# mitake/k8s

Hardware: AMD Instinct MI355X
Metric: images/sec ResNet-50 TfJob (train, synthetic ImageNet) (higher is better)
Workload: dtype bf16; 1 GPU; model=resnet50-v1.5, global_batch=3072, per_gpu_batch=3072, image_size=224, parallelism=dp1, optimizer=fused SGD momentum 0.9 (HIP)

## Files before the change

### k8s_amd/csrc/kernels/conv3x3.hip

```cpp
#include <stdexcept>

#include "common.h"
#include "launchers.h"
#include "mfma.h"

namespace k8s_amd {

namespace c3 {
constexpr int THREADS = 256;
constexpr int STAT_REPL = 32;
__device__ __attribute__((aligned(64))) uint16_t g_c3_zero[64];

__device__ __forceinline__ int swz(int p) { return p & 6; }

__device__ __forceinline__ void raw_barrier() {
  asm volatile("" ::: "memory");
  __builtin_amdgcn_s_barrier();
  asm volatile("" ::: "memory");
}

template <int W, int RT, int KT, bool XF>
struct Geo {
  static constexpr int WP = (W + 7) / 8 * 8 + (W % 8 == 0 ? 8 : 0), P = RT * W;
  static constexpr int NPOS = (RT + 2) * WP + 8;
  static constexpr int MF = (P + 31) / 32, NF = KT / 32;
  static constexpr int WIN_B = NPOS * 128, WT_B = KT * 128;
  static constexpr int NS = WIN_B + 3 * WT_B <= 80 * 1024 ? 3 : 2;
  static constexpr int STAGE_B = 32 * MF * KT * 2;
  static constexpr int LDS = (WIN_B + NS * WT_B) > STAGE_B ? (WIN_B + NS * WT_B) : STAGE_B;
  static_assert(WIN_B + NS * WT_B <= 80 * 1024, "two blocks per CU");
  static_assert(LDS >= THREADS * 16 * 4, "room for the statistics partials");
  static_assert(WP % 8 == 0 && WP > W, "pitch");
};

template <int W, int RT, int KT, bool XF>
__global__ void __launch_bounds__(THREADS, 2) conv3x3_kernel(const uint16_t* __restrict__ x,
                                                            const uint16_t* __restrict__ wt, uint16_t* __restrict__ y,
                                                            float* __restrict__ stats, const float* __restrict__ xf,
                                                            int H, int C, int K, int tiles_per_img, BnBwdSums bb) {
  using G = Geo<W, RT, KT, XF>;
  constexpr int WP = G::WP, NPOS = G::NPOS, P = G::P, MF = G::MF, NF = G::NF, NS = G::NS;
  constexpr int WOPS = KT * 8 / THREADS;
  __shared__ __attribute__((aligned(1024))) char smem[G::LDS];
  char* const win = smem;
  const int tid = threadIdx.x, lane = tid & 63;
  const int wid = __builtin_amdgcn_readfirstlane(tid >> 6);
  const int wm = wid >> 1, wn = wid & 1;
  const int tile = blockIdx.x;
  const int n = tile / tiles_per_img, h0 = (tile - n * tiles_per_img) * RT;
  const int k0 = blockIdx.y * KT;

  int pw[MF];
#pragma unroll
  for (int f = 0; f < MF; ++f) {
    const int m = (wm * MF + f) * 16 + (lane & 15), r = m / W;
    pw[f] = r * WP + 7 + (m - r * W);
  }
  int boff[2][NF];
#pragma unroll
  for (int kk = 0; kk < 2; ++kk)
#pragma unroll
    for (int j = 0; j < NF; ++j) {
      const int r = wn * (KT / 2) + j * 16 + (lane & 15), ch = kk * 4 + (lane >> 4);
      boff[kk][j] = r * 128 + ((ch ^ swz(r)) << 4);
    }
  f32x4_t acc[MF][NF];
#pragma unroll
  for (int f = 0; f < MF; ++f)
#pragma unroll
    for (int j = 0; j < NF; ++j) acc[f][j] = f32x4_t{0.f, 0.f, 0.f, 0.f};

  constexpr int PADR = WP - W, NPAD = 8 + (RT + 2) * PADR;
#pragma unroll
  for (int t0 = 0; t0 < NPAD * 8; t0 += THREADS) {
    const int t = t0 + tid, pi = t >> 3;
    if (t < NPAD * 8) {
      const int r = (pi - 8) / PADR;
      const int pos = pi < 8 ? pi : 8 + r * WP + W + (pi - 8 - r * PADR);
      *reinterpret_cast<bf16x8_t*>(win + (pos * 8 + (t & 7)) * 16) = bf16x8_t{0, 0, 0, 0, 0, 0, 0, 0};
    }
  }
  constexpr int IPR = (W * 8 + 63) / 64, NWI = (RT + 2) * IPR;
  const int lch = (lane & 7) ^ ((lane >> 3) & 6);
  const uint16_t* const xlane = x + ((long)n * H * W + (lane >> 3)) * C + lch * 8;
  auto load_window = [&](int c0) {
#pragma unroll 1
    for (int wi = wid; wi < NWI; wi += THREADS / 64) {
      const int wr = wi / IPR, i = wi - wr * IPR, h = h0 - 1 + wr;
      if (i * 8 + (lane >> 3) < W) {
        const void* src = (unsigned)h < (unsigned)H ? (const void*)(xlane + (h * W + i * 8) * C + c0)
                                                    : (const void*)g_c3_zero;
        glds16(src, win + (wr * WP + 8 + i * 8) * 128);
      }
    }
  };
  auto transform_window = [&](int c0) {
    const int lc = (tid & 7) ^ ((tid >> 3) & 6);
    float sc[8], sh[8];
#pragma unroll
    for (int j = 0; j < 8; ++j) {
      sc[j] = xf[c0 + lc * 8 + j];
      sh[j] = xf[C + c0 + lc * 8 + j];
    }
#pragma unroll 1
    for (int c = tid; c < NPOS * 8; c += THREADS) {
      const int q = (c >> 3) - 8, wr = q / WP, h = h0 - 1 + wr;
      if (q >= 0 && q - wr * WP < W && wr < RT + 2 && (unsigned)h < (unsigned)H) {
        bf16x8_t* qp = reinterpret_cast<bf16x8_t*>(win + c * 16);
        const bf16x8_t v = *qp;
        float o[8];
#pragma unroll
        for (int j = 0; j < 8; ++j) o[j] = fmaxf(__builtin_fmaf(bf2f((uint16_t)v[j]), sc[j], sh[j]), 0.f);
        *qp = pack_bf16x8(o);
      }
    }
    __syncthreads();
  };
  uint32_t wlane[WOPS];
#pragma unroll
  for (int i = 0; i < WOPS; ++i) {
    const int c = i * THREADS + tid, row = c >> 3, lc = (c & 7) ^ swz(row);
    wlane[i] = (uint32_t)(((k0 + row) * 9 * C + lc * 8) * 2);
  }
  auto stage_w = [&](int tap, int c0, int slot) {
    char* d = smem + G::WIN_B + slot * G::WT_B;
#pragma unroll
    for (int i = 0; i < WOPS; ++i) {
      glds16(reinterpret_cast<const char*>(wt + tap * C + c0) + wlane[i], d + (i * THREADS + wid * 64) * 16);
    }
  };
  auto tap_of = [](int k) { return (k % 3) * 3 + k / 3; };

  constexpr int CPR = KT / 8;
  constexpr int RSTEP = THREADS / CPR, NR = (P + RSTEP - 1) / RSTEP;
  constexpr bool XEARLY = KT == 64;
  const int c = tid % CPR, row0 = tid / CPR;
  const bool bst = bb.sums != nullptr;
  bf16x8_t xr[NR];
  auto load_xr = [&]() {
#pragma unroll
    for (int i = 0; i < NR; ++i) {
      const int m = row0 + i * RSTEP, hr = m / W, h = h0 + hr;
      xr[i] = bf16x8_t{0, 0, 0, 0, 0, 0, 0, 0};
      if (m < P && h < H)
        xr[i] = *reinterpret_cast<const bf16x8_t*>(bb.x + (((long)n * H + h) * W + (m - hr * W)) * K + k0 + c * 8);
    }
  };
  const int nsteps = (C >> 6) * 9;
  load_window(0);
  if (XEARLY && bst) load_xr();
#pragma unroll
  for (int g = 0; g < NS - 1; ++g)
    if (g < nsteps) stage_w(tap_of(g), 0, g);
  asm volatile("s_waitcnt vmcnt(0)" ::: "memory");
  __syncthreads();
  if constexpr (XF) transform_window(0);
#pragma unroll 1
  for (int cs = 0; cs < (C >> 6); ++cs) {
    if (cs) {
      load_window(cs * 64);
      asm volatile("s_waitcnt vmcnt(0)" ::: "memory");
      __syncthreads();
      if constexpr (XF) transform_window(cs * 64);
    }
#pragma unroll 1
    for (int ds = 0; ds < 3; ++ds) {
      int aoff[2][MF];
#pragma unroll
      for (int f = 0; f < MF; ++f) {
        const int p = pw[f] + ds;
#pragma unroll
        for (int kk = 0; kk < 2; ++kk) aoff[kk][f] = p * 128 + (((kk * 4 + (lane >> 4)) ^ swz(p)) << 4);
      }
#pragma unroll
      for (int dr = 0; dr < 3; ++dr) {
        const int g = cs * 9 + ds * 3 + dr, gp = g + NS - 1;
        if (gp < nsteps) stage_w(tap_of(gp % 9), gp / 9 * 64, gp % NS);
        const char* ws = smem + G::WIN_B + (NS == 3 ? dr : g & 1) * G::WT_B;
        const char* wa = win + dr * WP * 128;
        if constexpr (NF == 2) {
          mfma_bf16x8 af[2][MF], bfr[2][NF];
#pragma unroll
          for (int kk = 0; kk < 2; ++kk) {
#pragma unroll
            for (int f = 0; f < MF; ++f)
              af[kk][f] = __builtin_bit_cast(mfma_bf16x8, *reinterpret_cast<const bf16x8_t*>(wa + aoff[kk][f]));
#pragma unroll
            for (int j = 0; j < NF; ++j)
              bfr[kk][j] = __builtin_bit_cast(mfma_bf16x8, *reinterpret_cast<const bf16x8_t*>(ws + boff[kk][j]));
          }
          __builtin_amdgcn_sched_barrier(0);
#pragma unroll
          for (int kk = 0; kk < 2; ++kk) {
            if (kk == 0) asm volatile("s_waitcnt lgkmcnt(%0)" ::"n"(MF + NF) : "memory");
            else asm volatile("s_waitcnt lgkmcnt(0)" ::: "memory");
            __builtin_amdgcn_sched_barrier(0);
#pragma unroll
            for (int f = 0; f < MF; ++f)
#pragma unroll
              for (int j = 0; j < NF; ++j)
                acc[f][j] = __builtin_amdgcn_mfma_f32_16x16x32_bf16(bfr[kk][j], af[kk][f], acc[f][j], 0, 0, 0);
            __builtin_amdgcn_sched_barrier(0);
          }
        } else {
#pragma unroll
          for (int kk = 0; kk < 2; ++kk) {
            mfma_bf16x8 af[MF], bfr[NF];
#pragma unroll
            for (int f = 0; f < MF; ++f)
              af[f] = __builtin_bit_cast(mfma_bf16x8, *reinterpret_cast<const bf16x8_t*>(wa + aoff[kk][f]));
#pragma unroll
            for (int j = 0; j < NF; ++j)
              bfr[j] = __builtin_bit_cast(mfma_bf16x8, *reinterpret_cast<const bf16x8_t*>(ws + boff[kk][j]));
#pragma unroll
            for (int f = 0; f < MF; ++f)
#pragma unroll
              for (int j = 0; j < NF; ++j)
                acc[f][j] = __builtin_amdgcn_mfma_f32_16x16x32_bf16(bfr[j], af[f], acc[f][j], 0, 0, 0);
          }
        }
        if (NS > 2 && gp < nsteps) asm volatile("s_waitcnt vmcnt(%0)" ::"n"(WOPS * (NS - 2)) : "memory");
        else asm volatile("s_waitcnt vmcnt(0)" ::: "memory");
        asm volatile("s_waitcnt lgkmcnt(0)" ::: "memory");
        raw_barrier();
      }
    }
  }

  float bsc[8], bsh[8], bmu[8];
  if (bst) {
#pragma unroll
    for (int j = 0; j < 8; ++j) {
      const int col = k0 + c * 8 + j;
      bmu[j] = bb.mean[col];
      bn_affine_regs(bb.gamma[col], bb.beta[col], bmu[j], bb.invstd[col], bsc[j], bsh[j]);
    }
    if (!XEARLY) load_xr();
  }
  uint16_t* const ctile = reinterpret_cast<uint16_t*>(smem);
#pragma unroll
  for (int f = 0; f < MF; ++f) {
    const int row = (wm * MF + f) * 16 + (lane & 15);
#pragma unroll
    for (int j = 0; j < NF; ++j) {
      const int col = wn * (KT / 2) + j * 16 + (lane >> 4) * 4;
      const bf16x4_t o = __builtin_bit_cast(bf16x4_t, __builtin_convertvector(acc[f][j], bf16v4_t));
      *reinterpret_cast<bf16x4_t*>(ctile + row * KT + (((col >> 3) ^ (row % CPR)) << 3) + (col & 4)) = o;
    }
  }
  __syncthreads();
  f32x2_t s2[4], q2[4];
#pragma unroll
  for (int r = 0; r < 4; ++r) s2[r] = q2[r] = f32x2_t{0.f, 0.f};
  if (bst) {
#pragma unroll
    for (int i = 0; i < NR; ++i) {
      const int m = row0 + i * RSTEP, hr = m / W, h = h0 + hr;
      if (m < P && h < H) {
        const bf16x8_t o = *reinterpret_cast<const bf16x8_t*>(ctile + m * KT + ((c ^ (m % CPR)) << 3));
        *reinterpret_cast<bf16x8_t*>(y + (((long)n * H + h) * W + (m - hr * W)) * K + k0 + c * 8) = o;
#pragma unroll
        for (int r = 0; r < 4; ++r) {
          f32x2_t g, d;
#pragma unroll
          for (int e = 0; e < 2; ++e) {
            const float xv = bf2f((uint16_t)xr[i][2 * r + e]);
            g[e] = relu_on(xv, bsc[2 * r + e], bsh[2 * r + e]) ? bf2f((uint16_t)o[2 * r + e]) : 0.f;
            d[e] = xv - bmu[2 * r + e];
          }
          s2[r] += g;
          q2[r] = __builtin_elementwise_fma(g, d, q2[r]);
        }
      }
    }
  } else {
#pragma unroll 2
  for (int m = row0; m < P; m += RSTEP) {
    const int hr = m / W, h = h0 + hr;
    if (h < H) {
      const bf16x8_t o = *reinterpret_cast<const bf16x8_t*>(ctile + m * KT + ((c ^ (m % CPR)) << 3));
      *reinterpret_cast<bf16x8_t*>(y + (((long)n * H + h) * W + (m - hr * W)) * K + k0 + c * 8) = o;
      if (stats) {
        const uint32_t* w = reinterpret_cast<const uint32_t*>(&o);
#pragma unroll
        for (int r = 0; r < 4; ++r) {
          const f32x2_t v = {__uint_as_float(w[r] << 16), __uint_as_float(w[r] & 0xFFFF0000u)};
          s2[r] += v;
          q2[r] = __builtin_elementwise_fma(v, v, q2[r]);
        }
      }
    }
  }
  }
  if (stats || bst) {
    __syncthreads();
    float* part = reinterpret_cast<float*>(smem);
#pragma unroll
    for (int r = 0; r < 4; ++r) {
      part[tid * 16 + 2 * r] = s2[r][0];
      part[tid * 16 + 2 * r + 1] = s2[r][1];
      part[tid * 16 + 8 + 2 * r] = q2[r][0];
      part[tid * 16 + 8 + 2 * r + 1] = q2[r][1];
    }
    __syncthreads();
    if (tid < 2 * KT) {
      const int col = tid % KT, which = tid / KT, cc = col >> 3, r = col & 7;
      float v = 0.f;
#pragma unroll 4
      for (int t = cc; t < THREADS; t += CPR) v += part[t * 16 + which * 8 + r];
      atomicAdd((bst ? bb.sums : stats) + (long)(tile % STAT_REPL) * 2 * K + (long)which * K + k0 + col, v);
    }
  }
}


template <int W, int RT, int KT, bool XF>
static void launch(const uint16_t* x, const uint16_t* w, uint16_t* y, float* stats, const float* xf, int N, int H,
                   int C, int K, hipStream_t st, const BnBwdSums& bb) {
  const int tpi = (H + RT - 1) / RT;
  hipLaunchKernelGGL((conv3x3_kernel<W, RT, KT, XF>), dim3(N * tpi, K / KT), dim3(THREADS), 0, st, x, w, y, stats, xf,
                     H, C, K, tpi, bb);
}

template <int W, int RT, int KT>
static void launch_x(const uint16_t* x, const uint16_t* w, uint16_t* y, float* stats, const float* xf, int N, int H,
                     int C, int K, hipStream_t st, const BnBwdSums& bb) {
  if (xf) launch<W, RT, KT, true>(x, w, y, stats, xf, N, H, C, K, st, bb);
  else launch<W, RT, KT, false>(x, w, y, stats, xf, N, H, C, K, st, bb);
}
}

bool conv3x3_eligible(int H, int W, int C, int K, int R, int S, int stride, int pad, int dil) {
  const char* e = getenv("K8S_AMD_CONV3X3");
  if (e && e[0] == '0') return false;
  if (R != 3 || S != 3 || stride != 1 || pad != 1 || dil != 1 || H != W || C % 64 != 0) return false;
  if (W == 56) return K == 64;
  return (W == 28 || W == 14) && K % 128 == 0;
}

void launch_conv3x3(const uint16_t* x, const uint16_t* w, uint16_t* y, float* stats, const float* xform, int N,
                    int H, int W, int C, int K, hipStream_t st, const BnBwdSums* bsums) {
  const BnBwdSums bb = bsums ? *bsums : BnBwdSums{};
  if (bb.sums && (stats || !bb.x || !bb.gamma || !bb.beta || !bb.mean || !bb.invstd))
    throw std::runtime_error("conv3x3: BatchNorm-backward sums need x / gamma / beta / mean / invstd, no statistics");
  if (W == 56 && K == 64) c3::launch_x<56, 4, 64>(x, w, y, stats, xform, N, H, C, K, st, bb);
  else if (W == 28 && K % 128 == 0) c3::launch_x<28, 8, 128>(x, w, y, stats, xform, N, H, C, K, st, bb);
  else if (W == 14 && K % 128 == 0) c3::launch_x<14, 14, 128>(x, w, y, stats, xform, N, H, C, K, st, bb);
  else throw std::runtime_error("conv3x3: shape outside the staged-window kernel's contract");
}

}
```

Measured before the change: 16730 images/s.

## Use window-pitch position order for conv3x3 tiles and group blocks by adjacent tiles

For the 28x28 and 14x14 3x3 convolutions, output rows are now indexed at the padded window pitch (a power of two), so each lane's A-operand LDS address is a plain offset. A compile-time bank model asserts that A and B reads take four LDS cycles with no conflicts. Padding columns are computed and then masked at store time. A second option remaps the grid so the K panels of eight neighbouring tiles are launched together, meant to improve L2 reuse of the input windows. The cost is some wasted MFMA work on padding positions, and the 28x28 case changes to 7 rows per tile.

```diff
diff --git a/k8s_amd/csrc/kernels/conv3x3.hip b/k8s_amd/csrc/kernels/conv3x3.hip
--- a/k8s_amd/csrc/kernels/conv3x3.hip
+++ b/k8s_amd/csrc/kernels/conv3x3.hip
@@ -1,3 +1,5 @@
+#include <cstdlib>
+#include <cstring>
 #include <stdexcept>
 
 #include "common.h"
@@ -11,18 +13,25 @@
 constexpr int STAT_REPL = 32;
 __device__ __attribute__((aligned(64))) uint16_t g_c3_zero[64];
 
-__device__ __forceinline__ int swz(int p) { return p & 6; }
-
 __device__ __forceinline__ void raw_barrier() {
   asm volatile("" ::: "memory");
   __builtin_amdgcn_s_barrier();
   asm volatile("" ::: "memory");
 }
 
-template <int W, int RT, int KT, bool XF>
+constexpr int swz(int p) { return p & 6; }
+constexpr int log2i(int v) { return v <= 1 ? 0 : 1 + log2i(v >> 1); }
+constexpr int lane_group(int lane) {
+  const int l = lane & 31;
+  return (lane >> 5) * 2 + ((l < 4 || (l >= 12 && l < 16) || (l >= 20 && l < 28)) ? 0 : 1);
+}
+
+template <int W, int RT, int KT, bool XF, bool PO = false>
 struct Geo {
-  static constexpr int WP = (W + 7) / 8 * 8 + (W % 8 == 0 ? 8 : 0), P = RT * W;
-  static constexpr int NPOS = (RT + 2) * WP + 8;
+  static constexpr int WP = (W + 7) / 8 * 8 + (W % 8 == 0 ? 8 : 0);
+  static constexpr int PITCH = PO ? WP : W;
+  static constexpr int P = RT * PITCH;
+  static constexpr int NPOS = (RT + 2) * WP + 8 + (PO ? 8 : 0);
   static constexpr int MF = (P + 31) / 32, NF = KT / 32;
   static constexpr int WIN_B = NPOS * 128, WT_B = KT * 128;
   static constexpr int NS = WIN_B + 3 * WT_B <= 80 * 1024 ? 3 : 2;
@@ -31,14 +40,52 @@
   static_assert(WIN_B + NS * WT_B <= 80 * 1024, "two blocks per CU");
   static_assert(LDS >= THREADS * 16 * 4, "room for the statistics partials");
   static_assert(WP % 8 == 0 && WP > W, "pitch");
+  static_assert(!PO || ((WP & (WP - 1)) == 0 && P == MF * 32), "position order: shifts, and no partial fragment");
+  static_assert(!PO || 7 + P - 1 + 2 * WP + 2 < NPOS, "position order: every lane reads inside the window");
+
+  static constexpr int row_of(int m) { return PO ? m >> log2i(WP) : m / W; }
+  static constexpr int col_of(int m) { return PO ? m & (WP - 1) : m - m / W * W; }
+  static constexpr int pos_of_row(int m) { return PO ? 7 + m : row_of(m) * WP + 7 + col_of(m); }
+  static constexpr int a_off(int p, int kk, int lane) { return p * 128 + (((kk * 4 + (lane >> 4)) ^ swz(p)) << 4); }
+  static constexpr int b_off(int r, int kk, int lane) { return r * 128 + (((kk * 4 + (lane >> 4)) ^ swz(r)) << 4); }
+  static constexpr int a_row(int wm, int f, int lane) { return (wm * MF + f) * 16 + (lane & 15); }
+  static constexpr int b_row(int wn, int j, int lane) { return wn * (KT / 2) + j * 16 + (lane & 15); }
+
+  template <class F>
+  static constexpr int read_cycles(F off) {
+    int cnt[4][16] = {}, mx[4] = {}, cyc = 0;
+    for (int l = 0; l < 64; ++l) {
+      const int g = lane_group(l), n = ++cnt[g][(off(l) >> 4) & 15];
+      if (n > mx[g]) mx[g] = n;
+    }
+    for (int g = 0; g < 4; ++g) cyc += mx[g];
+    return cyc;
+  }
+  static constexpr bool reads_conflict_free() {
+    for (int kk = 0; kk < 2; ++kk) {
+      for (int wm = 0; wm < 2; ++wm)
+        for (int f = 0; f < MF; ++f)
+          for (int ds = 0; ds < 3; ++ds)
+            if (read_cycles([=](int l) { return a_off(pos_of_row(a_row(wm, f, l)) + ds, kk, l); }) != 4) return false;
+      for (int wn = 0; wn < 2; ++wn)
+        for (int j = 0; j < NF; ++j)
+          if (read_cycles([=](int l) { return b_off(b_row(wn, j, l), kk, l); }) != 4) return false;
+    }
+    return true;
+  }
+  static_assert(WIN_B % 256 == 0 && WT_B % 256 == 0, "operand images keep their bank phase");
 };
-
-template <int W, int RT, int KT, bool XF>
+static_assert(Geo<28, 7, 128, false, true>::reads_conflict_free(), "28 x 28: 4 LDS cycles per A and B read");
+static_assert(Geo<14, 14, 128, false, true>::reads_conflict_free(), "14 x 14: 4 LDS cycles per A and B read");
+static_assert(!Geo<14, 14, 128, false, false>::reads_conflict_free(), "the bank model sees the row order's conflicts");
+
+template <int W, int RT, int KT, bool XF, bool PO>
 __global__ void __launch_bounds__(THREADS, 2) conv3x3_kernel(const uint16_t* __restrict__ x,
                                                             const uint16_t* __restrict__ wt, uint16_t* __restrict__ y,
                                                             float* __restrict__ stats, const float* __restrict__ xf,
-                                                            int H, int C, int K, int tiles_per_img, BnBwdSums bb) {
-  using G = Geo<W, RT, KT, XF>;
+                                                            int H, int C, int K, int tiles_per_img, int adj_tiles,
+                                                            BnBwdSums bb) {
+  using G = Geo<W, RT, KT, XF, PO>;
   constexpr int WP = G::WP, NPOS = G::NPOS, P = G::P, MF = G::MF, NF = G::NF, NS = G::NS;
   constexpr int WOPS = KT * 8 / THREADS;
   __shared__ __attribute__((aligned(1024))) char smem[G::LDS];
@@ -46,37 +93,36 @@
   const int tid = threadIdx.x, lane = tid & 63;
   const int wid = __builtin_amdgcn_readfirstlane(tid >> 6);
   const int wm = wid >> 1, wn = wid & 1;
-  const int tile = blockIdx.x;
+  int tile = blockIdx.x, k0 = blockIdx.y * KT;
+  if (adj_tiles) {
+    const int gsz = 8 * (K / KT), grp = blockIdx.x / gsz, in = blockIdx.x - grp * gsz;
+    tile = grp * 8 + (in & 7);
+    k0 = (in >> 3) * KT;
+    if (tile >= adj_tiles) return;
+  }
   const int n = tile / tiles_per_img, h0 = (tile - n * tiles_per_img) * RT;
-  const int k0 = blockIdx.y * KT;
 
   int pw[MF];
 #pragma unroll
-  for (int f = 0; f < MF; ++f) {
-    const int m = (wm * MF + f) * 16 + (lane & 15), r = m / W;
-    pw[f] = r * WP + 7 + (m - r * W);
-  }
+  for (int f = 0; f < MF; ++f) pw[f] = G::pos_of_row(G::a_row(wm, f, lane));
   int boff[2][NF];
 #pragma unroll
   for (int kk = 0; kk < 2; ++kk)
 #pragma unroll
-    for (int j = 0; j < NF; ++j) {
-      const int r = wn * (KT / 2) + j * 16 + (lane & 15), ch = kk * 4 + (lane >> 4);
-      boff[kk][j] = r * 128 + ((ch ^ swz(r)) << 4);
-    }
+    for (int j = 0; j < NF; ++j) boff[kk][j] = G::b_off(G::b_row(wn, j, lane), kk, lane);
   f32x4_t acc[MF][NF];
 #pragma unroll
   for (int f = 0; f < MF; ++f)
 #pragma unroll
     for (int j = 0; j < NF; ++j) acc[f][j] = f32x4_t{0.f, 0.f, 0.f, 0.f};
 
-  constexpr int PADR = WP - W, NPAD = 8 + (RT + 2) * PADR;
+  constexpr int PADR = WP - W, NPADR = 8 + (RT + 2) * PADR, NPAD = NPADR + (PO ? 8 : 0);
 #pragma unroll
   for (int t0 = 0; t0 < NPAD * 8; t0 += THREADS) {
     const int t = t0 + tid, pi = t >> 3;
     if (t < NPAD * 8) {
       const int r = (pi - 8) / PADR;
-      const int pos = pi < 8 ? pi : 8 + r * WP + W + (pi - 8 - r * PADR);
+      const int pos = pi < 8 ? pi : pi >= NPADR ? NPOS - 8 + (pi - NPADR) : 8 + r * WP + W + (pi - 8 - r * PADR);
       *reinterpret_cast<bf16x8_t*>(win + (pos * 8 + (t & 7)) * 16) = bf16x8_t{0, 0, 0, 0, 0, 0, 0, 0};
     }
   }
@@ -137,13 +183,16 @@
   const int c = tid % CPR, row0 = tid / CPR;
   const bool bst = bb.sums != nullptr;
   bf16x8_t xr[NR];
+  auto pixel = [&](int m) -> long {
+    const int h = h0 + G::row_of(m), col = G::col_of(m);
+    return m < P && h < H && col < W ? (((long)n * H + h) * W + col) * K + k0 + c * 8 : -1;
+  };
   auto load_xr = [&]() {
 #pragma unroll
     for (int i = 0; i < NR; ++i) {
-      const int m = row0 + i * RSTEP, hr = m / W, h = h0 + hr;
+      const long o = pixel(row0 + i * RSTEP);
       xr[i] = bf16x8_t{0, 0, 0, 0, 0, 0, 0, 0};
-      if (m < P && h < H)
-        xr[i] = *reinterpret_cast<const bf16x8_t*>(bb.x + (((long)n * H + h) * W + (m - hr * W)) * K + k0 + c * 8);
+      if (o >= 0) xr[i] = *reinterpret_cast<const bf16x8_t*>(bb.x + o);
     }
   };
   const int nsteps = (C >> 6) * 9;
@@ -168,9 +217,11 @@
       int aoff[2][MF];
 #pragma unroll
       for (int f = 0; f < MF; ++f) {
-        const int p = pw[f] + ds;
-#pragma unroll
-        for (int kk = 0; kk < 2; ++kk) aoff[kk][f] = p * 128 + (((kk * 4 + (lane >> 4)) ^ swz(p)) << 4);
+#pragma unroll
+        for (int kk = 0; kk < 2; ++kk) {
+          if constexpr (PO) aoff[kk][f] = G::a_off(pw[0] + ds, kk, lane) + f * 16 * 128;
+          else aoff[kk][f] = G::a_off(pw[f] + ds, kk, lane);
+        }
       }
 #pragma unroll
       for (int dr = 0; dr < 3; ++dr) {
@@ -255,10 +306,11 @@
   if (bst) {
 #pragma unroll
     for (int i = 0; i < NR; ++i) {
-      const int m = row0 + i * RSTEP, hr = m / W, h = h0 + hr;
-      if (m < P && h < H) {
+      const int m = row0 + i * RSTEP;
+      const long po = pixel(m);
+      if (po >= 0) {
         const bf16x8_t o = *reinterpret_cast<const bf16x8_t*>(ctile + m * KT + ((c ^ (m % CPR)) << 3));
-        *reinterpret_cast<bf16x8_t*>(y + (((long)n * H + h) * W + (m - hr * W)) * K + k0 + c * 8) = o;
+        *reinterpret_cast<bf16x8_t*>(y + po) = o;
 #pragma unroll
         for (int r = 0; r < 4; ++r) {
           f32x2_t g, d;
@@ -276,10 +328,10 @@
   } else {
 #pragma unroll 2
   for (int m = row0; m < P; m += RSTEP) {
-    const int hr = m / W, h = h0 + hr;
-    if (h < H) {
+    const long po = pixel(m);
+    if (po >= 0) {
       const bf16x8_t o = *reinterpret_cast<const bf16x8_t*>(ctile + m * KT + ((c ^ (m % CPR)) << 3));
-      *reinterpret_cast<bf16x8_t*>(y + (((long)n * H + h) * W + (m - hr * W)) * K + k0 + c * 8) = o;
+      *reinterpret_cast<bf16x8_t*>(y + po) = o;
       if (stats) {
         const uint32_t* w = reinterpret_cast<const uint32_t*>(&o);
 #pragma unroll
@@ -313,20 +365,28 @@
   }
 }
 
-
-template <int W, int RT, int KT, bool XF>
+template <int W, int RT, int KT, bool XF, bool PO>
 static void launch(const uint16_t* x, const uint16_t* w, uint16_t* y, float* stats, const float* xf, int N, int H,
-                   int C, int K, hipStream_t st, const BnBwdSums& bb) {
-  const int tpi = (H + RT - 1) / RT;
-  hipLaunchKernelGGL((conv3x3_kernel<W, RT, KT, XF>), dim3(N * tpi, K / KT), dim3(THREADS), 0, st, x, w, y, stats, xf,
-                     H, C, K, tpi, bb);
-}
-
-template <int W, int RT, int KT>
+                   int C, int K, hipStream_t st, const BnBwdSums& bb, bool adjacent) {
+  const int tpi = (H + RT - 1) / RT, tiles = N * tpi, panels = K / KT;
+  const dim3 grid = adjacent ? dim3((tiles + 7) / 8 * 8 * panels) : dim3(tiles, panels);
+  hipLaunchKernelGGL((conv3x3_kernel<W, RT, KT, XF, PO>), grid, dim3(THREADS), 0, st, x, w, y, stats, xf, H, C, K,
+                     tpi, adjacent ? tiles : 0, bb);
+}
+
+template <int W, int RT, int KT, bool PO = false>
 static void launch_x(const uint16_t* x, const uint16_t* w, uint16_t* y, float* stats, const float* xf, int N, int H,
-                     int C, int K, hipStream_t st, const BnBwdSums& bb) {
-  if (xf) launch<W, RT, KT, true>(x, w, y, stats, xf, N, H, C, K, st, bb);
-  else launch<W, RT, KT, false>(x, w, y, stats, xf, N, H, C, K, st, bb);
+                     int C, int K, hipStream_t st, const BnBwdSums& bb, bool adjacent = false) {
+  if (xf) launch<W, RT, KT, true, PO>(x, w, y, stats, xf, N, H, C, K, st, bb, adjacent);
+  else launch<W, RT, KT, false, PO>(x, w, y, stats, xf, N, H, C, K, st, bb, adjacent);
+}
+
+enum class Order { Row, Pos, PosAdjacent };
+static Order order() {
+  const char* e = getenv("K8S_AMD_C3_ORDER");
+  if (e && !strcmp(e, "row")) return Order::Row;
+  if (e && !strcmp(e, "pos")) return Order::Pos;
+  return Order::PosAdjacent;
 }
 }
 
@@ -343,8 +403,12 @@
   const BnBwdSums bb = bsums ? *bsums : BnBwdSums{};
   if (bb.sums && (stats || !bb.x || !bb.gamma || !bb.beta || !bb.mean || !bb.invstd))
     throw std::runtime_error("conv3x3: BatchNorm-backward sums need x / gamma / beta / mean / invstd, no statistics");
+  const c3::Order ord = c3::order();
+  const bool po = ord != c3::Order::Row, adj = ord == c3::Order::PosAdjacent && K > 128;
   if (W == 56 && K == 64) c3::launch_x<56, 4, 64>(x, w, y, stats, xform, N, H, C, K, st, bb);
+  else if (W == 28 && K % 128 == 0 && po) c3::launch_x<28, 7, 128, true>(x, w, y, stats, xform, N, H, C, K, st, bb, adj);
   else if (W == 28 && K % 128 == 0) c3::launch_x<28, 8, 128>(x, w, y, stats, xform, N, H, C, K, st, bb);
+  else if (W == 14 && K % 128 == 0 && po) c3::launch_x<14, 14, 128, true>(x, w, y, stats, xform, N, H, C, K, st, bb, adj);
   else if (W == 14 && K % 128 == 0) c3::launch_x<14, 14, 128>(x, w, y, stats, xform, N, H, C, K, st, bb);
   else throw std::runtime_error("conv3x3: shape outside the staged-window kernel's contract");
 }
```

New measurement: 16780 images/s, median of 5. About the same (+0.3%).
